# subtotechnoblade/Grok_Alpha_Zero

Measured on NVIDIA B200. Metric: MCTS simulations/sec, higher is better.
Workload: dtype bf16

## Files before the change

### grok_alpha_zero_b200/csrc/gaz_block.cuh

```cuda
#pragma once
#include "gaz_conv.cuh"

#ifdef GAZ_BLOCK_CLK
#define TK_BEGIN() do { if (dbg & 1024) tq = clock64(); } while (0)
#define TK_END(acc) do { if (dbg & 1024) acc += clock64() - tq; } while (0)
#define TK_PRINT(...) printf(__VA_ARGS__)
#define TK_START(v) v = clock64()
#define TK_STOP(v) v = clock64() - v
#else
#define TK_START(v) do { } while (0)
#define TK_STOP(v) do { } while (0)
#define TK_BEGIN() do { } while (0)
#define TK_END(acc) do { } while (0)
#define TK_PRINT(...) do { } while (0)
#endif

namespace gaz_block {
using namespace gaz_tc;
using gaz_conv::f32_blk_index;
using gaz_conv::HALO;
using gaz_conv::ldg256;
using gaz_conv::named_bar_sync;
using gaz_conv::Ring;
using gaz_conv::SLAB_BOX_ROWS;
// ... 378 lines not shown
                named_bar_sync(2, 128);
            }
            for (int lt = pair0; lt < n_loop; lt += pair_step, it++) {
                const bool work = (2 * lt + rank) < n_tiles && !e1_off;
                TK_BEGIN();
#pragma unroll 1
                for (int h = 0; h < 2; h++) {
                    const int pos = h * 128 + e1_q * 32 + lane;
                    const int bp = pos % p.P_pad, yy = bp / p.Wp;
                    const bool live = yy != 0 && yy <= p.H && (bp % p.Wp) != p.Wp - 1 && (2 * lt + rank) * bpt + pos / p.P_pad < cnt;
                    const uint32_t t_sub = tmem_base + ((uint32_t)(e1_q * 32) << 16) + (uint32_t)((it & 1) * 2 * BN + h * BN);
                    e1_half(&acc1_full[h], &e1_done[h], (uint32_t)(it & 1), work, t_sub, par_addr, sH_addr, HALO + pos, live, lane);
                }
                TK_END(tk_work);
            }
        }
        if ((dbg & 1024) && blockIdx.x == 0 && warp == 4 && lane == 0) TK_PRINT("epilogue1: wait + work %lld\n", tk_work);
    } else if (warp >= 8) {
        const int ew = warp - 8;
        const int q = warp & 3, sub = ew >> 2;
        const int et = threadIdx.x - 256;
        float *s_part = s_se, *s_mean = s_se + 8 * BN, *s_hp = s_mean + BN, *s_h = s_hp + 256, *s_gate = s_h + 64, *s_bg = s_gate + BN;
        float *s_gp = s_part;
        const float inv_cells = 1.0f / (float)p.n_cells;
        const int pos = sub * 128 + q * 32 + lane;
        const int bp = pos % p.P_pad;
        const bool live_pos = (bp / p.Wp) != 0 && (bp / p.Wp) <= p.H && (bp % p.Wp) != p.Wp - 1;
        const uint32_t gate_addr = smem_u32(s_gate), bg_addr = smem_u32(s_bg);
        const uint32_t stage_addr = smem_u32(sStage + ew * 2 * 2048);
        int it = 0;
        [[maybe_unused]] long long tk_wait = 0, tk_se = 0, tk_out = 0, tq = 0;
        for (int l = 0; l < NL; l++) {
            const TrunkLayer &L = p.L[l];
            const bool use_res = L.res && !(dbg & 8);
            const bool do_se = L.se && !(dbg & 64);
            if (!do_se) {
                named_bar_sync(1, 256);
                if (et < BN) { s_gate[et] = 1.0f; s_bg[et] = L.par2[et]; }
                named_bar_sync(1, 256);
            }
            for (int lt = pair0; lt < n_loop; lt += pair_step, it++) {
                const int t = 2 * lt + rank;
                const int as = it & 1;
                const uint32_t sph = (uint32_t)((it >> 1) & 1);
                if (t >= n_tiles) {
                    mbar_wait(&acc2_full[as], sph);
                    tc_fence_before();
                    __syncwarp();
                    if (lane == 0) { mbar_arrive_leader(&acc2_empty[as]); s_done[ew] = it + 1; }
                    continue;
                }
                const size_t rbase = ((size_t)(t * 8 + sub * 4 + q) << 12) + (size_t)(lane * 8);
                const float *resp = L.res + rbase;
                float *outp = L.out_raw + rbase;
                const int row0 = t * TILE_ROWS + sub * 128 + q * 32;
                const bool live = live_pos && t * bpt + pos / p.P_pad < cnt;
                const uint32_t mask = live ? 0xffffffffu : 0u;
                float resA[16], resB[16];
                if (use_res) {
#pragma unroll 1
                    for (int k = 4; k < 16; k++) asm volatile("prefetch.global.L2 [%0];" ::"l"(resp + k * 256));
                    ldg256(resp, *reinterpret_cast<float(*)[8]>(&resA[0]));
                    ldg256(resp + 256, *reinterpret_cast<float(*)[8]>(&resA[8]));
                }
                TK_BEGIN();
                mbar_wait(&acc2_full[as], sph);
                TK_END(tk_wait);
                tc_fence_after();
                const uint32_t t_acc = tmem_base + ((uint32_t)(q * 32) << 16) + (uint32_t)(as * 2 * BN + sub * BN);
                TK_BEGIN();
                if (do_se) {
                    {
                        uint32_t ra[32], rb[32];
                        float *dst = s_part + ew * BN;
                        tmem_ld_32x32(t_acc, ra);
#pragma unroll 1
                        for (int h = 0; h < 2; h++) {
                            tmem_ld_wait_dep(ra);
                            tmem_ld_32x32(t_acc + (uint32_t)(h * 64 + 32), rb);
                            colsum32(ra, mask, lane, dst + h * 64);
                            tmem_ld_wait_dep(rb);
                            if (h == 0) tmem_ld_32x32(t_acc + 64u, ra);
                            colsum32(rb, mask, lane, dst + h * 64 + 32);
                        }
                    }
                    named_bar_sync(1, 256);
                    if (et < BN) {
                        float sum = 0.0f;
#pragma unroll
                        for (int k = 0; k < 8; k++) sum += s_part[k * BN + et];
                        s_mean[et] = sum * inv_cells;
                    }
                    named_bar_sync(1, 256);
                    {
                        const int j = et & 63, part = et >> 6;
                        if (j < L.se_r) {
                            const float *w1 = L.se_w1 + (size_t)(part * 32) * L.se_r + j;
                            const float4 *m4 = reinterpret_cast<const float4 *>(s_mean + part * 32);
                            float h0 = 0.0f, h1 = 0.0f, h2 = 0.0f, h3 = 0.0f;
#pragma unroll
                            for (int i = 0; i < 8; i++) {
                                const float4 m = m4[i];
                                h0 = fmaf(m.x, __ldg(w1 + (size_t)(4 * i) * L.se_r), h0);
                                h1 = fmaf(m.y, __ldg(w1 + (size_t)(4 * i + 1) * L.se_r), h1);
                                h2 = fmaf(m.z, __ldg(w1 + (size_t)(4 * i + 2) * L.se_r), h2);
                                h3 = fmaf(m.w, __ldg(w1 + (size_t)(4 * i + 3) * L.se_r), h3);
                            }
// ... 79 lines not shown
```

### grok_alpha_zero_b200/csrc/gaz_net.cu

```cuda
#include "../../include/gaz_net.h"
#include "gaz_internal.h"
#include "gaz_tc.cuh"
#include "gaz_conv.cuh"
#include "gaz_block.cuh"
#include "gaz_stem.cuh"
#include "gaz_small.cuh"

#include <cuda_bf16.h>
#include <math.h>
#include <stdio.h>

using namespace gaz_tc;
using gaz_conv::f32_blk_index;

#define CKN(x)                                                                                             \
    do {                                                                                                   \
        cudaError_t _e = (x);                                                                              \
        if (_e != cudaSuccess) return gaz_fail("%s: %s (%s:%d)", #x, cudaGetErrorString(_e), __FILE__, __LINE__); \
    } while (0)

struct SeArgs {
    const int32_t *count;
    int max_count, H, W, C, R, P_pad, Wp;
    const float *c2;
// ... 276 lines not shown
    const int leaf = (blockIdx.x * blockDim.x + threadIdx.x) >> 5, lane = threadIdx.x & 31;
    if (leaf >= cnt) return;
    const float *lg = logits + (size_t)leaf * P;
    float *po = policy + (size_t)leaf * P;
    if (mode == GAZ_POLICY_LINEAR) {
        for (int i = lane; i < P; i += 32) po[i] = lg[i];
        return;
    }
    if (mode == GAZ_POLICY_SOFTMAX) {
        double mx = -1e300;
        for (int i = lane; i < P; i += 32) mx = fmax(mx, (double)lg[i]);
        for (int o = 16; o > 0; o >>= 1) mx = fmax(mx, __shfl_xor_sync(0xffffffffu, mx, o));
        double s = 0.0;
        for (int i = lane; i < P; i += 32) s += exp((double)lg[i] - mx);
        for (int o = 16; o > 0; o >>= 1) s += __shfl_xor_sync(0xffffffffu, s, o);
        for (int i = lane; i < P; i += 32) po[i] = (float)(exp((double)lg[i] - mx) / s);
        return;
    }
    float s = 0.0f;
    for (int i = lane; i < P; i += 32) {
        float x = lg[i];
        s += x >= 0.0f ? x + 1.0f : 1.0f / (1.0f - x);
    }
    for (int o = 16; o > 0; o >>= 1) s += __shfl_xor_sync(0xffffffffu, s, o);
    for (int i = lane; i < P; i += 32) {
        float x = lg[i];
        po[i] = (x >= 0.0f ? x + 1.0f : 1.0f / (1.0f - x)) / s;
    }
}

__global__ void set_count_kernel(int32_t *c, int v) { *c = v; }
__global__ void chunk_count_kernel(const int32_t *total, int offset, int max, int32_t *out) {
    int c = *total - offset;
    *out = c < 0 ? 0 : (c > max ? max : c);
}

typedef CUresult (*PFN_encodeTiled)(CUtensorMap *, CUtensorMapDataType, cuuint32_t, void *, const cuuint64_t *,
                                    const cuuint64_t *, const cuuint32_t *, const cuuint32_t *, CUtensorMapInterleave,
                                    CUtensorMapSwizzle, CUtensorMapL2promotion, CUtensorMapFloatOOBfill);

struct NetBuf { int kind, width; void *ptr; size_t bytes; };
struct NetOp {
    gaz_net_op d;
    CUtensorMap tmA2;
    CUtensorMap tmB2;
    CUtensorMap tmOa, tmOb;
    int fused_se;
    gaz_net_op se;
    int skip;
    int block_fused;
    int in_block;
    int trunk_len;
    int in_trunk;
    int dxm;
    int dual_partner;
    int dual_skip;
    int head_wide;
    int head_tc;
    __nv_bfloat16 *d_xbf;
    uint4 *d_frag;
    float *d_hbias;
    int head_G;
    int chain_len;
    int chain_skip;
    uint4 *d_frag0;
    int chain_partner;
    int chain_joined;
    float par[5 * 128];
    float *d_se_b1;
    int dense_tc;
    __nv_bfloat16 *d_act;
    __nv_bfloat16 *d_wt;
    int stem_tc;
    int stem_tile;
    int stem_proj;
    uint16_t *d_stem_w;
    float *d_stem_par;
    CUtensorMap tmDA, tmDW2;
    long long rows_dense;
};

struct gaz_net {
    int game, H, W, Cin, P, Wp, P_pad, max_batch, policy_mode, device;
    long long rows_alloc;
    std::vector<NetBuf> bufs;
    std::vector<NetOp> ops;
    float *wf;
    uint16_t *wh;
    int64_t bytes;
    int n_sm;
    cudaStream_t stream;
    cudaStream_t stream2;
    cudaEvent_t ev_fork, ev_join;
    gaz_block::TrunkArgs *trunk_args;
    int head1_begin, head2_begin;
    int8_t *d_states;
    int32_t *d_count;
    int32_t *d_chunk_count;
    float *d_policy, *d_value;
    int logits_buf;
    int profile;
    int dbg;
    std::vector<cudaEvent_t> ev;
    size_t ev_used;
    std::vector<int> ev_op;
};
// ... 7 lines not shown
    CUresult r = enc(m, CU_TENSOR_MAP_DATA_TYPE_BFLOAT16, 2, ptr, dims, strides, box, estr, CU_TENSOR_MAP_INTERLEAVE_NONE,
                     sw, CU_TENSOR_MAP_L2_PROMOTION_L2_256B, CU_TENSOR_MAP_FLOAT_OOB_FILL_NONE);
    if (r != CUDA_SUCCESS) return gaz_fail("cuTensorMapEncodeTiled failed (%d) inner=%llu rows=%llu box=%ux%u", (int)r,
                                           (unsigned long long)inner, (unsigned long long)rows, box_inner, box_rows);
    return 0;
}
static int make_map(PFN_encodeTiled enc, CUtensorMap *m, void *ptr, uint64_t inner, uint64_t rows, uint32_t box_rows) {
    return make_map_ex(enc, m, ptr, inner, rows, 64, box_rows, CU_TENSOR_MAP_SWIZZLE_128B);
}

template <int BN> static int launch_conv_board(gaz_net *n, NetOp &op, const gaz_conv::BoardConvArgs &a, cudaStream_t s) {
    static bool attr_set = false;
    if (!attr_set) {
        CKN(cudaFuncSetAttribute(gaz_conv::conv_board_kernel<BN, true>, cudaFuncAttributeMaxDynamicSharedMemorySize,
                                 gaz_conv::BoardCfg<BN, true>::SMEM));
        attr_set = true;
    }
    cudaLaunchConfig_t cfg;
    memset(&cfg, 0, sizeof cfg);
    cfg.gridDim = dim3((unsigned)(n->n_sm & ~1), 1, 1);
    cfg.blockDim = dim3(384, 1, 1);
    cfg.dynamicSmemBytes = gaz_conv::BoardCfg<BN, true>::SMEM;
    cfg.stream = s;
    cudaLaunchAttribute at[1];
    at[0].id = cudaLaunchAttributeClusterDimension;
    at[0].val.clusterDim.x = 2; at[0].val.clusterDim.y = 1; at[0].val.clusterDim.z = 1;
    cfg.attrs = at;
    cfg.numAttrs = 1;
    CKN(cudaLaunchKernelEx(&cfg, gaz_conv::conv_board_kernel<BN, true>, op.tmA2, op.tmB2, op.tmOa, op.tmOb, a));
    return 0;
}

static int launch_res_trunk(gaz_net *n, size_t first, const int32_t *count, cudaStream_t s) {
    static bool attr_set = false;
    if (!attr_set) {
        CKN(cudaFuncSetAttribute(gaz_block::res_trunk_kernel, cudaFuncAttributeMaxDynamicSharedMemorySize, gaz_block::Cfg::SMEM));
        attr_set = true;
    }
    auto buf = [&](int id) -> void * { return id < 0 ? nullptr : n->bufs[(size_t)id].ptr; };
    gaz_block::TrunkArgs &a = *n->trunk_args;
    memset(&a, 0, sizeof a);
    a.count = count; a.max_count = n->max_batch; a.Wp = n->Wp; a.H = n->H; a.P_pad = n->P_pad; a.n_cells = n->H * n->W; a.dbg = n->dbg;
    a.n_layers = n->ops[first].trunk_len;
    size_t oi = first;
    for (int l = 0; l < a.n_layers; l++) {
        NetOp &c1 = n->ops[oi], &c2 = n->ops[oi + 1];
        gaz_block::TrunkLayer &L = a.L[l];
        L.tmA = c1.tmA2; L.tmW1 = c1.tmB2; L.tmW2 = c2.tmB2; L.tmOa = c2.tmOa; L.tmOb = c2.tmOb;
        L.nkc1 = c1.d.cin / 64;
        L.dep = l > 0;
        memcpy(L.par1, c1.par, sizeof L.par1);
        memcpy(L.par2, c2.par, sizeof L.par2);
        const gaz_net_op &o = c2.fused_se ? c2.se : c2.d;
        L.res = (const float *)buf(o.res_buf); L.out_raw = (float *)buf(o.out_raw);
        L.out_a = (__nv_bfloat16 *)buf(o.out_a); L.out_b = (__nv_bfloat16 *)buf(o.out_b);
        if (c2.d_xbf) { L.out_a = c2.d_xbf; L.plain_a = 1; }
        if (c2.fused_se) {
            L.se = 1; L.se_r = c2.se.cin;
            L.se_w1 = n->wf + c2.se.w2; L.se_b1 = c2.d_se_b1; L.se_w2 = n->wf + c2.se.w3; L.se_b2 = n->wf + c2.se.bias3;
        }
        oi += c2.fused_se ? 3 : 2;
    }
    cudaLaunchConfig_t cfg;
    memset(&cfg, 0, sizeof cfg);
    cfg.gridDim = dim3((unsigned)(n->n_sm & ~1), 1, 1);
    cfg.blockDim = dim3(512, 1, 1);
    cfg.dynamicSmemBytes = gaz_block::Cfg::SMEM;
    cfg.stream = s;
    cudaLaunchAttribute at[1];
    at[0].id = cudaLaunchAttributeClusterDimension;
    at[0].val.clusterDim.x = 2; at[0].val.clusterDim.y = 1; at[0].val.clusterDim.z = 1;
    cfg.attrs = at;
    cfg.numAttrs = 1;
    CKN(cudaLaunchKernelEx(&cfg, gaz_block::res_trunk_kernel, a));
    return 0;
}

static const float *wfp(gaz_net *n, int64_t off) { return off < 0 ? nullptr : n->wf + off; }

static int net_forward(gaz_net *n, const int8_t *states, const int32_t *count, float *policy, float *value, cudaStream_t s_main) {
    n->ev_used = n->profile ? n->ev_used : 0;
    const bool two = n->head2_begin > 0;
    for (size_t oi = 0; oi < n->ops.size(); oi++) {
        if (two && (int)oi == n->head1_begin) {
            CKN(cudaEventRecord(n->ev_fork, s_main));
            CKN(cudaStreamWaitEvent(n->stream2, n->ev_fork, 0));
        }
        cudaStream_t s = (two && (int)oi >= n->head2_begin) ? n->stream2 : s_main;
        NetOp &op = n->ops[oi];
        const gaz_net_op &d = op.d;
        auto buf = [&](int id) -> void * { return id < 0 ? nullptr : n->bufs[(size_t)id].ptr; };
        switch (d.type) {
        case GAZ_OP_STEM: {
            if (op.stem_proj) {
                static bool attr_set = false;
                if (!attr_set) {
                    CKN(cudaFuncSetAttribute(gaz_stem::stem_proj_kernel, cudaFuncAttributeMaxDynamicSharedMemorySize, gaz_stem::ProjCfg::SMEM));
                    attr_set = true;
                }
                const gaz_net_op &pj = n->ops[oi + 1].d;
                gaz_stem::StemProjArgs t;
                t.count = count; t.max_count = n->max_batch; t.states = states; t.H = n->H; t.W = n->W; t.Wp = n->Wp;
                t.relu = d.act == GAZ_ACT_RELU; t.wpack = op.d_stem_w; t.par = op.d_stem_par;
                t.wproj = n->wh + pj.w; t.pbias = n->wf + pj.bias; t.out_res = (float *)buf(pj.out_raw);
                gaz_stem::stem_proj_kernel<<<n->n_sm, 512, gaz_stem::ProjCfg::SMEM, s>>>(op.tmOa, t);
                break;
            }
// ... 19 lines not shown
#define STEM_TILE(K_, C_)                                                                                                       \
    do {                                                                                                                        \
        const int sm = gaz_stem::TileCfg<K_, C_>::smem(n->H, n->W, n->P_pad);                                                    \
        static bool attr_set = false;                                                                                           \
        if (!attr_set) {                                                                                                        \
            CKN(cudaFuncSetAttribute(gaz_stem::stem_tile_kernel<K_, C_>, cudaFuncAttributeMaxDynamicSharedMemorySize, sm));      \
            attr_set = true;                                                                                                    \
        }                                                                                                                       \
        gaz_stem::stem_tile_kernel<K_, C_><<<grid, 256, sm, s>>>(op.tmOa, t);                                                    \
    } while (0)
                if (d.ksize == 3 && d.cin == 4) STEM_TILE(3, 4);
                else if (d.ksize == 3 && d.cin == 2) STEM_TILE(3, 2);
                else STEM_TILE(5, 2);
#undef STEM_TILE
                break;
            }
            {
                gaz_small::StemMmaArgs a;
                a.count = count; a.max_count = n->max_batch; a.states = states; a.H = n->H; a.W = n->W; a.Cout = d.cout;
                a.P_pad = n->P_pad; a.Wp = n->Wp; a.act = d.act; a.G = op.head_G; a.frags = op.d_frag; a.par = op.d_stem_par;
                a.out_q = (__nv_bfloat16 *)buf(d.out_b); a.out_raw = (float *)buf(d.out_raw); a.out_a = (__nv_bfloat16 *)buf(d.out_a);
                const int groups = (int)((n->rows_alloc / n->P_pad + a.G) / a.G);
                const int grid = groups < 2 * n->n_sm ? groups : 2 * n->n_sm;
                size_t sm;
#define STEM_MMA(K_, C_)                                                                                                        \
    do {                                                                                                                        \
        sm = gaz_small::StemMmaCfg<K_, C_>::smem(n->H, n->W, d.cout, a.G);                                                       \
        static bool attr_set = false;                                                                                           \
        if (!attr_set) {                                                                                                        \
            CKN(cudaFuncSetAttribute(gaz_small::stem_mma_kernel<K_, C_>, cudaFuncAttributeMaxDynamicSharedMemorySize, 96 * 1024)); \
            attr_set = true;                                                                                                    \
        }                                                                                                                       \
        if (sm > 96 * 1024) return gaz_fail("stem: %zu bytes of shared memory", sm);                                             \
        gaz_small::stem_mma_kernel<K_, C_><<<grid, 256, sm, s>>>(a);                                                             \
    } while (0)
                if (d.ksize == 3 && d.cin == 2) STEM_MMA(3, 2);
                else if (d.ksize == 3 && d.cin == 4) STEM_MMA(3, 4);
                else if (d.ksize == 5 && d.cin == 2) STEM_MMA(5, 2);
                else return gaz_fail("stem k=%d cin=%d unsupported", d.ksize, d.cin);
#undef STEM_MMA
            }
            break;
        }
        case GAZ_OP_CONV_TC: {
            if (op.in_block || op.in_trunk) break;
            if (n->profile && n->ev_used + 2 <= n->ev.size()) {
                n->ev_op.push_back((int)oi);
                CKN(cudaEventRecord(n->ev[n->ev_used++], s));
            }
            int rc;
            if (op.block_fused) {
                rc = launch_res_trunk(n, oi, count, s);
            } else {
                gaz_conv::BoardConvArgs a;
                memset(&a, 0, sizeof a);
                a.count = count; a.max_count = n->max_batch; a.P_pad = n->P_pad; a.Wp = n->Wp; a.H = n->H;
                a.taps = d.ksize * d.ksize; a.kpt = d.cin / 64; a.base_offset_mode = n->dbg;
                if (op.dxm) { a.taps = 3; a.dxm = 1; }
                const gaz_net_op &o = op.fused_se ? op.se : d;
                memcpy(a.par, op.par, sizeof a.par);
                a.res = (const float *)buf(o.res_buf); a.out_raw = (float *)buf(o.out_raw);
                a.out_a = (__nv_bfloat16 *)buf(o.out_a); a.out_b = (__nv_bfloat16 *)buf(o.out_b);
                if (op.fused_se) {
                    a.se = 1; a.se_r = op.se.cin; a.n_cells = n->H * n->W;
                    a.se_w1 = wfp(n, op.se.w2); a.se_b1 = wfp(n, op.se.bias2); a.se_w2 = wfp(n, op.se.w3); a.se_b2 = wfp(n, op.se.bias3);
                    a.se_b1 = op.d_se_b1;
                }
                rc = op.dxm ? launch_conv_board<96>(n, op, a, s)
                     : d.cout == 128 ? launch_conv_board<128>(n, op, a, s) : d.cout == 64 ? launch_conv_board<64>(n, op, a, s)
                     : d.cout == 32 ? launch_conv_board<32>(n, op, a, s) : gaz_fail("conv_tc cout %d unsupported", d.cout);
            }
            if (rc != 0) return rc;
            if (n->profile && (n->ev_used & 1)) CKN(cudaEventRecord(n->ev[n->ev_used++], s));
            break;
        }
        case GAZ_OP_SE: {
            if (op.skip) break;
            SeArgs a;
            a.count = count; a.max_count = n->max_batch; a.H = n->H; a.W = n->W; a.C = d.cout; a.R = d.cin;
            a.P_pad = n->P_pad; a.Wp = n->Wp;
            a.c2 = (const float *)buf(d.in_buf); a.res = (const float *)buf(d.res_buf);
            a.w1 = wfp(n, d.w2); a.b1 = wfp(n, d.bias2); a.w2 = wfp(n, d.w3); a.b2 = wfp(n, d.bias3);
            a.out_raw = (float *)buf(d.out_raw); a.out_a = (__nv_bfloat16 *)buf(d.out_a); a.out_b = (__nv_bfloat16 *)buf(d.out_b);
            a.scale_a = wfp(n, d.scale_a); a.shift_a = wfp(n, d.shift_a); a.scale_b = wfp(n, d.scale_b); a.shift_b = wfp(n, d.shift_b);
            if (d.cout != 128 || d.cin > 64) return gaz_fail("SE supports C=128, R<=64");
            se_kernel<<<n->n_sm * 16, 128, 0, s>>>(a);
            break;
        }
        case GAZ_OP_HEADCONV: {
            if (op.dual_skip) break;
            if (op.head_tc) {
                gaz_conv::BoardConvArgs a;
                memset(&a, 0, sizeof a);
                a.count = count; a.max_count = n->max_batch; a.P_pad = n->P_pad; a.Wp = n->Wp; a.H = n->H; a.W = n->W;
                a.taps = 3; a.kpt = d.cin / 64; a.dxm = 1; a.base_offset_mode = 0;
                memcpy(a.par, op.par, sizeof a.par);
                a.head_out[0] = (float *)buf(d.out_raw); a.head_c[0] = d.cout;
                if (op.dual_partner >= 0) {
                    const NetOp &o2 = n->ops[(size_t)op.dual_partner];
                    a.head_out[1] = (float *)buf(o2.d.out_raw); a.head_c[1] = o2.d.cout;
                }
                if (launch_conv_board<48>(n, op, a, s) != 0) return -1;
                break;
            }
            if (op.head_wide) {
                gaz_small::HeadWideArgs a;
// ... 151 lines not shown
    n->dbg = 0;
#ifdef GAZ_BLOCK_CLK
    { const char *e = getenv("GAZ_CONV_DBG"); n->dbg = e ? atoi(e) : 0; }
#endif
    n->profile = 0;
    n->ev_used = 0;
    n->logits_buf = -1;
    cudaDeviceProp prop;
    CKN(cudaGetDeviceProperties(&prop, desc->device));
    n->n_sm = prop.multiProcessorCount;
    CKN(cudaStreamCreateWithFlags(&n->stream, cudaStreamNonBlocking));
    CKN(cudaStreamCreateWithFlags(&n->stream2, cudaStreamNonBlocking));
    CKN(cudaEventCreateWithFlags(&n->ev_fork, cudaEventDisableTiming));
    CKN(cudaEventCreateWithFlags(&n->ev_join, cudaEventDisableTiming));
    n->head1_begin = 0; n->head2_begin = 0;
    n->trunk_args = new gaz_block::TrunkArgs();
    auto alloc = [&](void **p, size_t bytes) -> int {
        CKN(cudaMalloc(p, bytes ? bytes : 16));
        CKN(cudaMemset(*p, 0, bytes ? bytes : 16));
        n->bytes += (int64_t)bytes;
        return 0;
    };
    int rc = 0;
    rc |= alloc((void **)&n->wf, (size_t)desc->n_wf * 4);
    rc |= alloc((void **)&n->wh, (size_t)desc->n_wh * 2);
    if (rc == 0 && desc->n_wf) CKN(cudaMemcpy(n->wf, desc->wf, (size_t)desc->n_wf * 4, cudaMemcpyHostToDevice));
    if (rc == 0 && desc->n_wh) CKN(cudaMemcpy(n->wh, desc->wh, (size_t)desc->n_wh * 2, cudaMemcpyHostToDevice));
    for (int i = 0; i < desc->n_bufs && rc == 0; i++) {
        NetBuf b;
        b.kind = desc->bufs[i].kind;
        b.width = desc->bufs[i].width;
        if (b.kind == GAZ_BUF_ROWS_BF16) b.bytes = (size_t)n->rows_alloc * b.width * 2;
        else if (b.kind == GAZ_BUF_ROWS_F32) b.bytes = (size_t)n->rows_alloc * b.width * 4;
        else b.bytes = (size_t)n->max_batch * b.width * 4;
        b.ptr = nullptr;
        rc |= alloc(&b.ptr, b.bytes);
        n->bufs.push_back(b);
    }
    rc |= alloc((void **)&n->d_states, (size_t)n->max_batch * n->H * n->W * n->Cin);
    rc |= alloc((void **)&n->d_count, 16);
    rc |= alloc((void **)&n->d_chunk_count, 16 * 4);
    rc |= alloc((void **)&n->d_policy, (size_t)n->max_batch * n->P * 4);
    rc |= alloc((void **)&n->d_value, (size_t)n->max_batch * 4);
    if (rc != 0) { gaz_net_destroy(n); return -1; }
    for (int i = 0; i < desc->n_ops; i++) {
        NetOp op;
        op.d = desc->ops[i];
        memset(&op.tmA2, 0, sizeof op.tmA2);
        memset(&op.tmB2, 0, sizeof op.tmB2);
        op.fused_se = 0;
        op.skip = 0;
        op.block_fused = 0;
        op.in_block = 0;
        op.trunk_len = 0; op.in_trunk = 0;
        op.dxm = 0;
        op.dual_partner = -1;
        op.dual_skip = 0;
        op.head_tc = 0; op.d_xbf = nullptr;
        op.head_wide = 0; op.d_frag = nullptr; op.d_hbias = nullptr; op.head_G = 1; op.chain_len = 0; op.chain_skip = 0; op.chain_partner = -1; op.chain_joined = 0; op.d_frag0 = nullptr;
        op.stem_tc = 0;
        op.stem_tile = 0;
        op.stem_proj = 0;
        op.d_stem_w = nullptr;
        op.d_stem_par = nullptr;
        op.d_se_b1 = nullptr;
        op.dense_tc = 0; op.d_act = nullptr; op.d_wt = nullptr; op.rows_dense = 0;
        memset(&op.se, 0, sizeof op.se);
        const gaz_net_op &d = op.d;
        if (d.type == GAZ_OP_CONV_TC) {
            if (d.cin % 64 != 0 || (d.cout != 32 && d.cout != 64 && d.cout != 128) || (d.ksize != 1 && d.ksize != 3)) {
                gaz_net_destroy(n);
                return gaz_fail("conv_tc op %d: unsupported shape cin=%d cout=%d k=%d", i, d.cin, d.cout, d.ksize);
            }
            const NetBuf &ib = n->bufs[(size_t)d.in_buf];
            if (ib.kind != GAZ_BUF_ROWS_BF16 || ib.width != d.cin) {
                gaz_net_destroy(n);
                return gaz_fail("conv_tc op %d: input buffer must be bf16 rows of width cin", i);
            }
            if (make_map(enc, &op.tmA2, ib.ptr, (uint64_t)d.cin, (uint64_t)n->rows_alloc, gaz_conv::SLAB_BOX_ROWS) != 0 ||
                make_map(enc, &op.tmB2, n->wh + d.w, (uint64_t)d.ksize * d.ksize * d.cin, (uint64_t)d.cout, (uint32_t)d.cout / 2) != 0) {
                gaz_net_destroy(n);
                return -1;
            }
#ifndef GAZ_NO_DXM
            if (d.cout == 32 && d.ksize == 3 && gaz_conv::TILE_ROWS % n->P_pad == 0 && 32 % n->Wp == 0 && d.out_a >= 0 && d.out_b < 0 &&
                d.out_raw < 0 && d.res_buf < 0 && (n->n_sm & ~1) >= 2) {
                const size_t ld = (size_t)3 * d.cin;
                std::vector<uint16_t> wt((size_t)96 * ld);
                for (int dy = 0; dy < 3; dy++)
                    for (int dx = 0; dx < 3; dx++)
                        for (int c = 0; c < 32; c++)
                            memcpy(&wt[(size_t)(dx * 32 + c) * ld + (size_t)dy * d.cin], desc->wh + d.w + (size_t)c * 9 * d.cin + (size_t)(dy * 3 + dx) * d.cin,
                                   (size_t)d.cin * 2);
                if (alloc((void **)&op.d_wt, wt.size() * 2) != 0) { gaz_net_destroy(n); return -1; }
                CKN(cudaMemcpy(op.d_wt, wt.data(), wt.size() * 2, cudaMemcpyHostToDevice));
                if (make_map(enc, &op.tmB2, op.d_wt, (uint64_t)ld, 96, 48) != 0) { gaz_net_destroy(n); return -1; }
                op.dxm = 1;
            }
#endif
        }
        if (d.type == GAZ_OP_POLICY_OUT) n->logits_buf = d.in_buf;
        if (d.type == GAZ_OP_SE && n->P_pad == gaz_conv::TILE_ROWS && !n->ops.empty()) {
            NetOp &prev = n->ops.back();
            if (prev.d.type == GAZ_OP_CONV_TC && prev.d.out_raw == d.in_buf && prev.d.out_a < 0 && prev.d.out_b < 0 &&
                prev.d.res_buf < 0 && prev.d.cout == d.cout && d.cout == 128 && d.cin <= 64 && (d.cin & 1) == 0) {
                prev.fused_se = 1;
                prev.se = d;
// ... 138 lines not shown
                const gaz_net_op *dd = c < 8 ? &d1 : d2p;
                hb[c] = (dd && (c & 7) < dd->cout) ? desc->wf[dd->bias + (c & 7)] : 0.0f;
            }
            if (alloc((void **)&o1.d_frag, fr.size() * sizeof(gaz_small::Frag)) != 0 || alloc((void **)&o1.d_hbias, sizeof hb) != 0) { gaz_net_destroy(n); return -1; }
            CKN(cudaMemcpy(o1.d_frag, fr.data(), fr.size() * sizeof(gaz_small::Frag), cudaMemcpyHostToDevice));
            CKN(cudaMemcpy(o1.d_hbias, hb, sizeof hb, cudaMemcpyHostToDevice));
            o1.head_wide = 1;
            o1.head_G = G;
        }
    }
#ifndef GAZ_NO_HEAD_TC
    for (size_t i = 0; i < n->ops.size(); i++) {
        NetOp &o1 = n->ops[i];
        const gaz_net_op &d1 = o1.d;
        if (d1.type != GAZ_OP_HEADCONV || !o1.head_wide || d1.ksize != 3 || d1.cin != 128 || d1.cout > 8) continue;
        if (gaz_conv::TILE_ROWS % n->P_pad != 0 || 32 % n->Wp != 0 || (n->n_sm & ~1) < 2) continue;
        const gaz_net_op *d2p = o1.dual_partner >= 0 ? &n->ops[(size_t)o1.dual_partner].d : nullptr;
        NetOp *src = nullptr;
        for (auto &c2 : n->ops) {
            if (c2.d.type != GAZ_OP_CONV_TC || !c2.in_block) continue;
            const gaz_net_op &o = c2.fused_se ? c2.se : c2.d;
            if (o.out_raw == d1.in_buf && o.out_a < 0 && !c2.d_xbf) src = &c2;
        }
        if (!src) continue;
        if (alloc((void **)&src->d_xbf, (size_t)n->rows_alloc * 128 * 2) != 0) { gaz_net_destroy(n); return -1; }
        const size_t ld = (size_t)3 * d1.cin;
        std::vector<uint16_t> wt((size_t)48 * ld, 0);
        auto bf16_bits = [](float f) -> uint16_t { uint32_t u; memcpy(&u, &f, 4); return (uint16_t)((u + 0x7FFFu + ((u >> 16) & 1u)) >> 16); };
        for (int hd = 0; hd < 2; hd++) {
            const gaz_net_op *dd = hd == 0 ? &d1 : d2p;
            if (!dd) continue;
            for (int dy = 0; dy < 3; dy++)
                for (int dx = 0; dx < 3; dx++)
                    for (int k = 0; k < dd->cin; k++)
                        for (int c = 0; c < dd->cout; c++)
                            wt[(size_t)(dx * 16 + hd * 8 + c) * ld + (size_t)dy * dd->cin + k] =
                                bf16_bits(desc->wf[dd->w + ((int64_t)(dy * 3 + dx) * dd->cin + k) * dd->cout + c]);
        }
        if (alloc((void **)&o1.d_wt, wt.size() * 2) != 0) { gaz_net_destroy(n); return -1; }
        CKN(cudaMemcpy(o1.d_wt, wt.data(), wt.size() * 2, cudaMemcpyHostToDevice));
        if (make_map(enc, &o1.tmA2, src->d_xbf, 128, (uint64_t)n->rows_alloc, gaz_conv::SLAB_BOX_ROWS) != 0 ||
            make_map(enc, &o1.tmB2, o1.d_wt, (uint64_t)ld, 48, 24) != 0 ||
            make_map_ex(enc, &src->tmOa, src->d_xbf, 128, (uint64_t)n->rows_alloc, 32, 32, CU_TENSOR_MAP_SWIZZLE_64B) != 0) { gaz_net_destroy(n); return -1; }
        memset(&o1.tmOa, 0, sizeof o1.tmOa);
        memset(&o1.tmOb, 0, sizeof o1.tmOb);
        for (int c = 0; c < 640; c++) o1.par[c] = 0.0f;
        for (int c = 0; c < 16; c++) {
            const gaz_net_op *dd = c < 8 ? &d1 : d2p;
            o1.par[c] = (dd && (c & 7) < dd->cout) ? desc->wf[dd->bias + (c & 7)] : 0.0f;
        }
        o1.head_tc = 1;
    }
#endif
    for (size_t i = 0; i < n->ops.size(); i++) {
        NetOp &o1 = n->ops[i];
        if (o1.d.type != GAZ_OP_DENSE || o1.dense_tc || o1.chain_skip || o1.chain_len) continue;
        auto fits = [](const gaz_net_op &dd) { return dd.cin <= 512 && dd.cout <= 128; };
        if (!fits(o1.d)) continue;
        int len = 1;
        while (len < 3 && i + (size_t)len < n->ops.size()) {
            const NetOp &nx = n->ops[i + (size_t)len];
            const gaz_net_op &pv = n->ops[i + (size_t)len - 1].d;
            if (nx.d.type != GAZ_OP_DENSE || nx.dense_tc || !fits(nx.d) || (pv.flags & 4) || nx.d.in_buf != pv.out_raw || nx.d.cin != pv.cout) break;
            bool other = false;
            for (size_t k = 0; k < n->ops.size(); k++)
                if (k != i + (size_t)len && (n->ops[k].d.in_buf == pv.out_raw || n->ops[k].d.res_buf == pv.out_raw)) other = true;
            if (other || pv.out_raw == n->logits_buf) break;
            len++;
        }
        if (len < 2) continue;
        o1.chain_len = len;
        for (int k = 1; k < len; k++) n->ops[i + (size_t)k].chain_skip = 1;
    }
#ifndef GAZ_NO_MLP_MMA
    for (auto &o1 : n->ops) {
        const gaz_net_op &d = o1.d;
        if (d.type != GAZ_OP_DENSE || o1.dense_tc || o1.chain_skip || d.cin % 16 != 0 || d.cin < 128 || d.cin > 512) continue;
        if (o1.chain_len == 0) {
            if (d.cout < 64 || d.cout > 256) continue;
            o1.chain_len = 1;
        } else if (d.cout < 64 || d.cout > 128) continue;
        const int KS = d.cin / 16, NT = (((d.cout + 7) / 8) + 7) & ~7;
        std::vector<gaz_small::Frag> fr((size_t)KS * NT * 32);
        for (int ks = 0; ks < KS; ks++)
            for (int nt = 0; nt < NT; nt++)
                for (int lane = 0; lane < 32; lane++) {
                    auto wfun = [&](int k, int nn) -> float { return nn < d.cout ? desc->wf[d.w + (int64_t)k * d.cout + nn] : 0.0f; };
                    fr[((size_t)ks * NT + nt) * 32 + lane] = gaz_small::host_frag(lane, wfun, ks * 16, nt * 8);
                }
        if (alloc((void **)&o1.d_frag0, fr.size() * sizeof(gaz_small::Frag)) != 0) { gaz_net_destroy(n); return -1; }
        CKN(cudaMemcpy(o1.d_frag0, fr.data(), fr.size() * sizeof(gaz_small::Frag), cudaMemcpyHostToDevice));
    }
#endif
    for (size_t i = 0; i < n->ops.size(); i++) {
        NetOp &o1 = n->ops[i];
        if (o1.d.type != GAZ_OP_DENSE || o1.chain_len == 0 || o1.chain_joined || o1.chain_partner >= 0) continue;
        for (size_t j = i + (size_t)o1.chain_len; j < n->ops.size(); j++) {
            NetOp &o2 = n->ops[j];
            if (o2.d.type != GAZ_OP_DENSE || o2.chain_len == 0 || o2.chain_joined || o2.chain_partner >= 0) continue;
            bool ready = false, clash = false;
            for (size_t k = 0; k < n->ops.size(); k++) {
                const NetOp &pk = n->ops[k];
                if (pk.d.out_raw != o2.d.in_buf) continue;
                size_t exec = k;
                if (pk.dual_skip) { exec = n->ops.size(); for (size_t q = 0; q < k; q++) if (n->ops[q].dual_partner == (int)k) exec = q; }
                if (exec < i) ready = true; else clash = true;
// ... 355 lines not shown
```

### grok_alpha_zero_b200/net.py

```python
import ctypes as C

import numpy as np

from . import _lib
from ._net_symbols import GazNetBuf, GazNetDesc, GazNetOp
from .engine import GAMES, EngineError
from .netspec import bn_affine, is_tensor_core_conv, round_bf16

OP_STEM, OP_CONV_TC, OP_SE, OP_HEADCONV, OP_DENSE, OP_POLICY_OUT = range(6)
BUF_ROWS_BF16, BUF_ROWS_F32, BUF_FLAT_F32 = range(3)
ACT = {"none": 0, "relu": 1, "gelu": 2, "tanh": 3}
POLICY_MODE = {"softmax": 0, "stablemax": 1, "linear": 2}


def f32_to_bf16_bits(a):
    u = round_bf16(a).view(np.uint32)
    return (u >> 16).astype(np.uint16)


class _Builder:
    def __init__(self):
        self.wf = []
        self.n_wf = 0
        self.wh = []
        self.n_wh = 0
        self.bufs = []
        self.ops = []

    def f(self, arr):
        a = np.ascontiguousarray(arr, dtype=np.float32).reshape(-1)
        off = self.n_wf
        self.wf.append(a)
        self.n_wf += a.size
        pad = (-self.n_wf) % 4
        if pad:
            self.wf.append(np.zeros(pad, np.float32))
            self.n_wf += pad
        return off

    def h(self, arr):
        a = f32_to_bf16_bits(np.ascontiguousarray(arr, dtype=np.float32)).reshape(-1)
        off = self.n_wh
        self.wh.append(a)
        self.n_wh += a.size
        pad = (-self.n_wh) % 64
        if pad:
            self.wh.append(np.zeros(pad, np.uint16))
            self.n_wh += pad
        return off

    def buf(self, kind, width):
        self.bufs.append((kind, width))
        return len(self.bufs) - 1

    def op(self, type, **kw):
        d = dict(type=type, in_buf=-1, res_buf=-1, out_raw=-1, out_a=-1, out_b=-1, cin=0, cout=0, ksize=1, act=0,
                 flags=0, pad=0, w=-1, bias=-1, scale_a=-1, shift_a=-1, scale_b=-1, shift_b=-1, w2=-1, bias2=-1,
                 w3=-1, bias3=-1)
        d.update(kw)
        self.ops.append(d)


def build_ops(spec, W):
    B = _Builder()
    layers = spec["layers"]
    stem = layers[0]
    blocks = [l for l in layers if l["op"] == "block"]
    heads = [l for l in layers if l["op"] == "head"]
    F = blocks[0]["cout"]
    SF = stem["cout"]

    def aff(name):
        s, t = bn_affine(W, name)
        return B.f(s), B.f(t)

    def tc_weights(name, k):
        kern = W[name + ".kernel"]
        return B.h(np.transpose(kern, (3, 0, 1, 2)).reshape(kern.shape[3], -1))

    head_pre = []
    for hd in heads:
        hl = hd["layers"]
        if hl[0]["t"] == "bnrelu" and hl[1]["t"] == "conv" and is_tensor_core_conv(hl[1]["cin"], hl[1]["cout"]):
            head_pre.append((hd["name"], hl[0]["name"]))
    assert len(head_pre) <= 2

    a_x = B.buf(BUF_ROWS_BF16, F)
    a_h = B.buf(BUF_ROWS_BF16, F)
    res = [B.buf(BUF_ROWS_F32, F), B.buf(BUF_ROWS_F32, F)]
    use_se = any(b["se"] for b in blocks)
    c2buf = B.buf(BUF_ROWS_F32, F) if use_se else -1
    head_in = {name: B.buf(BUF_ROWS_BF16, F) for name, _ in head_pre}

    first = blocks[0]
    sa, ta = aff(first["name"] + ".bn1")
    ss, ts = aff(stem["bn"])
    if first["proj"]:
        a_stem = B.buf(BUF_ROWS_BF16, SF)
        q_stem = B.buf(BUF_ROWS_BF16, SF)
        B.op(OP_STEM, cin=stem["cin"], cout=SF, ksize=stem["k"], act=ACT[stem["act"]], w=B.f(W[stem["name"] + ".kernel"]),
             bias=B.f(W[stem["name"] + ".bias"]), scale_b=ss, shift_b=ts, out_b=q_stem, out_a=a_stem, scale_a=sa, shift_a=ta)
        ain, rin = a_stem, -1
    else:
        B.op(OP_STEM, cin=stem["cin"], cout=SF, ksize=stem["k"], act=ACT[stem["act"]], w=B.f(W[stem["name"] + ".kernel"]),
             bias=B.f(W[stem["name"] + ".bias"]), scale_b=ss, shift_b=ts, out_raw=res[0], out_a=a_x, scale_a=sa, shift_a=ta)
        ain, rin = a_x, res[0]
        q_stem = -1
    cur = 0 if rin == res[0] else -1
    for bi, b in enumerate(blocks):
        n = b["name"]
        if b["proj"]:
            tgt = res[0]
            B.op(OP_CONV_TC, in_buf=q_stem, out_raw=tgt, cin=b["cin"], cout=b["cout"], ksize=1,
                 w=tc_weights(n + ".proj", 1), bias=B.f(W[n + ".proj.bias"]))
            rin, cur = tgt, 0
        s2, t2 = aff(n + ".bn2")
        B.op(OP_CONV_TC, in_buf=ain, out_a=a_h, cin=b["cin"], cout=b["cout"], ksize=3, w=tc_weights(n + ".conv1", 3),
             bias=B.f(W[n + ".conv1.bias"]), scale_a=s2, shift_a=t2)
        rout = res[1 - cur]
        last = bi == len(blocks) - 1
        outs = {}
        if not last:
            sA, tA = aff(blocks[bi + 1]["name"] + ".bn1")
            outs = dict(out_a=a_x, scale_a=sA, shift_a=tA)
        else:
            for slot, (hname, bnname) in zip("ab", head_pre):
                sA, tA = aff(bnname)
                outs["out_" + slot] = head_in[hname]
                outs["scale_" + slot] = sA
                outs["shift_" + slot] = tA
        if b["se"]:
            B.op(OP_CONV_TC, in_buf=a_h, out_raw=c2buf, cin=b["cout"], cout=b["cout"], ksize=3,
                 w=tc_weights(n + ".conv2", 3), bias=B.f(W[n + ".conv2.bias"]))
            B.op(OP_SE, in_buf=c2buf, res_buf=rin, out_raw=rout, cin=b["cout"] // 2, cout=b["cout"],
                 w2=B.f(W[n + ".se1.kernel"]), bias2=B.f(W[n + ".se1.bias"]), w3=B.f(W[n + ".se2.kernel"]),
                 bias3=B.f(W[n + ".se2.bias"]), **outs)
        else:
            B.op(OP_CONV_TC, in_buf=a_h, res_buf=rin, out_raw=rout, cin=b["cout"], cout=b["cout"], ksize=3,
                 w=tc_weights(n + ".conv2", 3), bias=B.f(W[n + ".conv2.bias"]), **outs)
        ain, rin, cur = a_x, rout, 1 - cur
    x_raw = rin
    H, Wd = spec["H"], spec["W"]
# ... 27 lines not shown
        B.op(OP_HEADCONV, in_buf=cur_rows, out_raw=flat, cin=conv["cin"], cout=conv["cout"], ksize=conv["k"],
             w=B.f(kern), bias=B.f(bias))
        pend_aff, pend_relu = None, False
        dense_layers = [l for l in hl[i:] if l["t"] == "dense"]
        cur_flat = flat
        for l in hl[i:]:
            if l["t"] == "bnrelu":
                pend_aff, pend_relu = l["name"], True
            elif l["t"] == "relu":
                pend_relu = True
            elif l["t"] == "dense":
                is_last = l is dense_layers[-1]
                kw = dict(in_buf=cur_flat, cin=l["cin"], cout=l["cout"], w=B.f(W[l["name"] + ".kernel"]),
                          bias=B.f(W[l["name"] + ".bias"]))
                flags = 0
                if pend_aff is not None:
                    s, t = aff(pend_aff)
                    kw.update(scale_a=s, shift_a=t)
                    flags |= 1
                if pend_relu:
                    flags |= 2
                if is_last and hd["out"] == "value":
                    flags |= 4
                    kw["act"] = ACT["tanh"]
                else:
                    nb = B.buf(BUF_FLAT_F32, l["cout"])
                    kw["out_raw"] = nb
                    cur_flat = nb
                B.op(OP_DENSE, flags=flags, **kw)
                pend_aff, pend_relu = None, False
        if hd["out"] == "policy":
            B.op(OP_POLICY_OUT, in_buf=cur_flat)
    return B


def check_weights(spec, W):
    from .keras_bridge import expected_shapes
    want = expected_shapes(spec)
    for l in spec["layers"]:
        if l["op"] == "block" and l["se"]:
            r = l["cout"] // 2
            want.update({l["name"] + ".se1.kernel": (l["cout"], r), l["name"] + ".se1.bias": (r,),
                         l["name"] + ".se2.kernel": (r, l["cout"]), l["name"] + ".se2.bias": (l["cout"],)})
    for k, shp in want.items():
        if k not in W:
            raise ValueError("network weights: %r is missing (spec %s %s)" % (k, spec["game"], spec["cfg"]))
        if tuple(np.shape(W[k])) != tuple(shp):
            raise ValueError("network weights: %r has shape %s, the spec (%s %s) expects %s"
                             % (k, tuple(np.shape(W[k])), spec["game"], spec["cfg"], tuple(shp)))


class Net:

    def __init__(self, spec, weights, max_batch, device=0, lib=None):
        self.lib = lib if lib is not None else _lib.load()
        self.spec = spec
        self.H, self.W, self.Cin, self.P = spec["H"], spec["W"], spec["Cin"], spec["P"]
        self.max_batch = max_batch
        check_weights(spec, weights)
        b = build_ops(spec, weights)
        self.n_ops = len(b.ops)
        self.n_conv_tc = sum(1 for o in b.ops if o["type"] == OP_CONV_TC)
        self.conv_shapes = [(o["cin"], o["cout"], o["ksize"]) for o in b.ops if o["type"] == OP_CONV_TC]
        p_pad = (spec["H"] + 1) * (spec["W"] + 1)
        if p_pad <= 256:
            r = 16
            while r < p_pad:
                r <<= 1
            p_pad = r
        tile_is_board = p_pad == 256
        fuse_block = 256 % p_pad == 0
        self._op_shapes = []
        for i, o in enumerate(b.ops):
            tag = ""
            if o["type"] == OP_CONV_TC and i + 1 < len(b.ops) and b.ops[i + 1]["type"] == OP_SE and tile_is_board:
                tag = "se"
            self._op_shapes.append([o["type"], o["cin"], o["cout"], o["ksize"], tag])
        if fuse_block:
            for i in range(len(b.ops) - 1):
                o, o2 = b.ops[i], b.ops[i + 1]
                if o["type"] == OP_CONV_TC and o2["type"] == OP_CONV_TC and (o["cin"], o["cout"], o["ksize"]) in ((128, 128, 3), (256, 128, 3)) and \
                        (o2["cin"], o2["cout"], o2["ksize"]) == (128, 128, 3) and o["out_a"] >= 0 and o["out_b"] < 0 and \
                        o["out_raw"] < 0 and o["res_buf"] < 0 and o2["in_buf"] == o["out_a"] and self._op_shapes[i][4] == "":
                    self._op_shapes[i][4] = "block+" + self._op_shapes[i + 1][4]
                    self._op_shapes[i + 1][4] = "inblock"
        self._op_shapes = [tuple(x) for x in self._op_shapes]
        bufs = (GazNetBuf * len(b.bufs))(*[GazNetBuf(k, w) for k, w in b.bufs])
        ops = (GazNetOp * len(b.ops))(*[GazNetOp(**o) for o in b.ops])
        wf = np.concatenate(b.wf) if b.wf else np.zeros(4, np.float32)
        wh = np.concatenate(b.wh) if b.wh else np.zeros(64, np.uint16)
        desc = GazNetDesc(GAMES[spec["game"]], max_batch, len(b.bufs), len(b.ops), POLICY_MODE[spec["policy_head"]],
                          device, bufs, ops, wf.ctypes.data_as(C.c_void_p), wf.size, wh.ctypes.data_as(C.c_void_p),
                          wh.size)
        h = C.c_void_p()
        self._h = None
        rc = self.lib.gaz_net_create(C.byref(desc), C.byref(h))
        if rc < 0:
            raise EngineError(self.lib.gaz_last_error().decode())
        self._h = h
        self.n_launches = int(self.lib.gaz_net_launches_per_forward(h))
        shapes = [list(x) for x in self._op_shapes]
        for i, x in enumerate(shapes):
            if x[4].startswith("block"):
                nb = int(self.lib.gaz_net_op_blocks(h, i))
                x[4] = "intrunk" if nb == 0 else (x[4] + "*%d" % nb)
        self._op_shapes = [tuple(x) for x in shapes]

    def _ck(self, rc):
        if rc < 0:
            raise EngineError(self.lib.gaz_last_error().decode())
        return rc

    def close(self):
# ... 46 lines not shown
```

Measured before the change: 647,900.

## Run residual stream in place and skip dead fp32 raw outputs in fused trunk

```diff
diff --git a/grok_alpha_zero_b200/csrc/gaz_block.cuh b/grok_alpha_zero_b200/csrc/gaz_block.cuh
--- a/grok_alpha_zero_b200/csrc/gaz_block.cuh
+++ b/grok_alpha_zero_b200/csrc/gaz_block.cuh
@@ -454,7 +454,7 @@
                 }
                 const size_t rbase = ((size_t)(t * 8 + sub * 4 + q) << 12) + (size_t)(lane * 8);
                 const float *resp = L.res + rbase;
-                float *outp = L.out_raw + rbase;
+                float *outp = L.out_raw ? L.out_raw + rbase : nullptr;
                 const int row0 = t * TILE_ROWS + sub * 128 + q * 32;
                 const bool live = live_pos && t * bpt + pos / p.P_pad < cnt;
                 const uint32_t mask = live ? 0xffffffffu : 0u;
diff --git a/grok_alpha_zero_b200/csrc/gaz_net.cu b/grok_alpha_zero_b200/csrc/gaz_net.cu
--- a/grok_alpha_zero_b200/csrc/gaz_net.cu
+++ b/grok_alpha_zero_b200/csrc/gaz_net.cu
@@ -352,6 +352,7 @@
     int in_block;
     int trunk_len;
     int in_trunk;
+    int raw_dead;
     int dxm;
     int dual_partner;
     int dual_skip;
@@ -465,7 +466,7 @@
         memcpy(L.par1, c1.par, sizeof L.par1);
         memcpy(L.par2, c2.par, sizeof L.par2);
         const gaz_net_op &o = c2.fused_se ? c2.se : c2.d;
-        L.res = (const float *)buf(o.res_buf); L.out_raw = (float *)buf(o.out_raw);
+        L.res = (const float *)buf(o.res_buf); L.out_raw = c2.raw_dead ? nullptr : (float *)buf(o.out_raw);
         L.out_a = (__nv_bfloat16 *)buf(o.out_a); L.out_b = (__nv_bfloat16 *)buf(o.out_b);
         if (c2.d_xbf) { L.out_a = c2.d_xbf; L.plain_a = 1; }
         if (c2.fused_se) {
@@ -591,6 +592,8 @@
             if (op.block_fused) {
                 rc = launch_res_trunk(n, oi, count, s);
             } else {
+                const gaz_net_op &io = op.fused_se ? op.se : d;
+                if (io.res_buf >= 0 && io.res_buf == io.out_raw) return gaz_fail("op %zu: an in-place residual stream needs the fused block kernel", oi);
                 gaz_conv::BoardConvArgs a;
                 memset(&a, 0, sizeof a);
                 a.count = count; a.max_count = n->max_batch; a.P_pad = n->P_pad; a.Wp = n->Wp; a.H = n->H;
@@ -848,7 +851,7 @@
         op.skip = 0;
         op.block_fused = 0;
         op.in_block = 0;
-        op.trunk_len = 0; op.in_trunk = 0;
+        op.trunk_len = 0; op.in_trunk = 0; op.raw_dead = 0;
         op.dxm = 0;
         op.dual_partner = -1;
         op.dual_skip = 0;
@@ -1093,6 +1096,23 @@
         o1.head_tc = 1;
     }
 #endif
+    for (size_t oi = 0; oi < n->ops.size(); oi++) {
+        NetOp &c2 = n->ops[oi];
+        if (c2.d.type != GAZ_OP_CONV_TC || !c2.in_block || oi == 0 || !n->ops[oi - 1].block_fused) continue;
+        const gaz_net_op &o = c2.fused_se ? c2.se : c2.d;
+        if (o.out_raw < 0) continue;
+        bool read = false;
+        for (size_t k = oi + (c2.fused_se ? 2 : 1); k < n->ops.size() && !read; k++) {
+            const NetOp &r = n->ops[k];
+            bool in_read = !(r.d.type == GAZ_OP_CONV_TC && r.in_block && k > 0 && n->ops[k - 1].block_fused) && !(r.d.type == GAZ_OP_SE && r.skip);
+            if (r.d.type == GAZ_OP_HEADCONV) {
+                if (r.head_tc) in_read = false;
+                for (size_t q = 0; q < k; q++) if (n->ops[q].dual_partner == (int)k && n->ops[q].head_tc) in_read = false;
+            }
+            if ((in_read && r.d.in_buf == o.out_raw) || r.d.res_buf == o.out_raw) read = true;
+        }
+        c2.raw_dead = read ? 0 : 1;
+    }
     for (size_t i = 0; i < n->ops.size(); i++) {
         NetOp &o1 = n->ops[i];
         if (o1.d.type != GAZ_OP_DENSE || o1.dense_tc || o1.chain_skip || o1.chain_len) continue;
diff --git a/grok_alpha_zero_b200/net.py b/grok_alpha_zero_b200/net.py
--- a/grok_alpha_zero_b200/net.py
+++ b/grok_alpha_zero_b200/net.py
@@ -61,7 +61,7 @@
         self.ops.append(d)
 
 
-def build_ops(spec, W):
+def build_ops(spec, W, stream_in_place=True):
     B = _Builder()
     layers = spec["layers"]
     stem = layers[0]
@@ -85,9 +85,16 @@
             head_pre.append((hd["name"], hl[0]["name"]))
     assert len(head_pre) <= 2
 
+    p_pad = (spec["H"] + 1) * (spec["W"] + 1)
+    if p_pad <= 256:
+        r = 16
+        while r < p_pad:
+            r <<= 1
+        p_pad = r
+    in_place = stream_in_place and 256 % p_pad == 0 and all(b["cin"] in (128, 256) and b["cout"] == 128 for b in blocks)
     a_x = B.buf(BUF_ROWS_BF16, F)
     a_h = B.buf(BUF_ROWS_BF16, F)
-    res = [B.buf(BUF_ROWS_F32, F), B.buf(BUF_ROWS_F32, F)]
+    res = [B.buf(BUF_ROWS_F32, F)] * 2 if in_place else [B.buf(BUF_ROWS_F32, F), B.buf(BUF_ROWS_F32, F)]
     use_se = any(b["se"] for b in blocks)
     c2buf = B.buf(BUF_ROWS_F32, F) if use_se else -1
     head_in = {name: B.buf(BUF_ROWS_BF16, F) for name, _ in head_pre}
@@ -221,13 +228,13 @@
 
 class Net:
 
-    def __init__(self, spec, weights, max_batch, device=0, lib=None):
+    def __init__(self, spec, weights, max_batch, device=0, lib=None, stream_in_place=True):
         self.lib = lib if lib is not None else _lib.load()
         self.spec = spec
         self.H, self.W, self.Cin, self.P = spec["H"], spec["W"], spec["Cin"], spec["P"]
         self.max_batch = max_batch
         check_weights(spec, weights)
-        b = build_ops(spec, weights)
+        b = build_ops(spec, weights, stream_in_place)
         self.n_ops = len(b.ops)
         self.n_conv_tc = sum(1 for o in b.ops if o["type"] == OP_CONV_TC)
         self.conv_shapes = [(o["cin"], o["cout"], o["ksize"]) for o in b.ops if o["type"] == OP_CONV_TC]
```

After: 653,800, median of 6. About the same (+0.9%).
